# 2thleZ/flash_attention_metal

Hardware: AMD Instinct MI355X
Metric: attn_fwd_tflops (seqlen=4096, head_dim=64, bf16, causal) (higher is better)
Workload: dtype bf16; 1 GPU; BASELINE.json configs[2]: seqlen=4096 head_dim=64 batch=4 heads=16 bf16 is_causal=true per GPU; batch_per_gpu=4, heads=16, seq_len=4096, head_dim=64, is_causal=True

## Files before the change

flash_attention_metal_amd/csrc/fa_mfma16_kernel.hip:

```cpp
#include <stdlib.h>

#include <algorithm>

#include "fa_mfma_common.h"

#ifndef FA16_DEFER_THR
#define FA16_DEFER_THR 8.0f
#endif
#ifndef FA16_LAK
#define FA16_LAK (D == 128 ? 3 : 2)
#endif
#ifndef FA16_LAV
#define FA16_LAV (D == 128 ? 3 : 2)
#endif
#ifndef FA16_PRIO
#define FA16_PRIO 1
#endif
#ifndef FA16_ONES
#define FA16_ONES 1
#endif
#ifndef FA16_HALVES
#define FA16_HALVES 0
#endif
#ifndef FA16_BN128
#define FA16_BN128 64
#endif
#ifndef FA16_OCC128
#define FA16_OCC128 2
#endif
#ifndef FA16_SUB8
#define FA16_SUB8 1
#endif
#ifndef FA16_OCC
#define FA16_OCC 4
#endif

namespace fa {

typedef float f32x4 __attribute__((ext_vector_type(4)));

template <typename Tag> struct MT16;
template <> struct MT16<BF16> {
  using elem = __bf16;
  using vec8 = bf16x8;
  __device__ static __forceinline__ f32x4 mfma(vec8 a, vec8 b, f32x4 c) { return __builtin_amdgcn_mfma_f32_16x16x32_bf16(a, b, c, 0, 0, 0); }
};
template <> struct MT16<F16> {
  using elem = _Float16;
  using vec8 = f16x8;
  __device__ static __forceinline__ f32x4 mfma(vec8 a, vec8 b, f32x4 c) { return __builtin_amdgcn_mfma_f32_16x16x32_f16(a, b, c, 0, 0, 0); }
};

__device__ __forceinline__ float xlane(float x, int mask) { return __shfl_xor(x, mask, 64); }

template <typename Tag, int D, bool CAUSAL, int RW, bool PAD, int SUB>
__device__ __forceinline__ void fwd_mfma16_body(const Params &p) {
  using M = MT16<Tag>;
  using vec8 = typename M::vec8;
  using elem = typename M::elem;
  constexpr int BMR = RW * WM;
  constexpr int RB = D * 2;
  constexpr int CPR = D / 8;
  constexpr int KS = D / 32;
  constexpr int DT = D / 16;
  constexpr int BNK = (D == 128) ? FA16_BN128 : BN;
  constexpr int KT = BNK / 16;
  constexpr int NKP = KT / 2;
  constexpr int TILE = BNK * RB;
  static_assert(D == 64 || D == 128, "head dims of the 16x16x32 kernel");

  extern __shared__ __attribute__((aligned(16))) char smem_generic[];
  lds_char *smem = (lds_char *)smem_generic;
  lds_char *Kbuf = smem;
  lds_char *Vbuf = smem + 2 * SUB * TILE;

  const int wave = __builtin_amdgcn_readfirstlane((int)threadIdx.x >> 6);
  const int lane = threadIdx.x & 63;
  const int c = lane & 15;
  const int g = lane >> 4;

  int bh, qb;
  map_block<CAUSAL>(blockIdx.x, p, bh, qb);
  long long base, base_kv;
  head_bases(bh, p, base, base_kv);
  const int coff = p.Nk - p.N;
  const int q0 = qb * BMR;
  const int qw0 = q0 + wave * WM;

  const int GRB = PAD ? p.D * 2 : RB;
  auto gcol = [&](int chunk) -> unsigned { return (!PAD || chunk * 8 < p.D) ? (unsigned)chunk * 16 : 0x80000000u; };
  const unsigned head_bytes = (unsigned)p.N * GRB, kv_head_bytes = (unsigned)p.Nk * GRB;
  const __amdgpu_buffer_rsrc_t rq = __builtin_amdgcn_make_buffer_rsrc((void *)((const char *)p.q + base * 2), 0, head_bytes, 0x00020000);
  const __amdgpu_buffer_rsrc_t rk = __builtin_amdgcn_make_buffer_rsrc((void *)((const char *)p.k + base_kv * 2), 0, kv_head_bytes, 0x00020000);
  const __amdgpu_buffer_rsrc_t rv = __builtin_amdgcn_make_buffer_rsrc((void *)((const char *)p.v + base_kv * 2), 0, kv_head_bytes, 0x00020000);

  vec8 qf[2][KS];
#pragma unroll
  for (int qt = 0; qt < 2; ++qt)
#pragma unroll
    for (int ks = 0; ks < KS; ++ks) {
      const u32x4 t = __builtin_amdgcn_raw_buffer_load_b128(rq, (unsigned)(qw0 + 16 * qt + c) * GRB + gcol(4 * ks + g), 0, 0);
      qf[qt][ks] = __builtin_bit_cast(vec8, t);
    }

  const int kx = (D == 64) ? ((c >> 1) & 7) : c;
  const lds_char *kptr[KS];
#pragma unroll
  for (int ks = 0; ks < KS; ++ks) {
    kptr[ks] = Kbuf + c * RB + (((4 * ks + g) ^ kx) << 4);
    asm volatile("" : "+v"(kptr[ks]));
  }
  const int vq = c >> 2, vp = c & 3;
  const int vrow = 4 * g + vq;
  const int vx = (D == 64) ? (((vrow >> 1) & 3) << 1) : ((vrow & 7) << 1);
  const lds_char *vptr[DT];
#pragma unroll
  for (int dt = 0; dt < DT; ++dt) {
    vptr[dt] = Vbuf + vrow * RB + ((((2 * dt) ^ vx) + (vp >> 1)) << 4) + 8 * (vp & 1);
    asm volatile("" : "+v"(vptr[dt]));
  }

  const int kv_end = CAUSAL ? min(p.Nk, q0 + BMR + coff) : p.Nk;
  const int nT = (kv_end + BNK - 1) / BNK;

  constexpr int RPP = 1024 / RB;
  constexpr int NPW = (BNK / RPP) / RW;
  static_assert((RW * RPP) % 16 == 0, "the piece stride must keep the swizzle");
  unsigned dma_kvo, dma_vvo;
  {
    const int row = wave * RPP + lane / CPR, pc = lane % CPR;
    const int skx = (D == 64) ? ((row >> 1) & 7) : (row & 15);
    const int svx = (D == 64) ? (((row >> 1) & 3) << 1) : ((row & 7) << 1);
    dma_kvo = (unsigned)(row * GRB) + gcol(pc ^ skx);
    dma_vvo = (unsigned)(row * GRB) + gcol(pc ^ svx);
  }
  auto stage_dma = [&](int t, int buf) {
#pragma unroll
    for (int j = 0; j < NPW; ++j) {
      const unsigned soff = PAD ? (unsigned)(t * BNK + j * RW * RPP) * GRB : (unsigned)t * TILE + j * (RW * 1024);
      const unsigned lk = (unsigned)(__UINTPTR_TYPE__)Kbuf + buf * TILE + (wave + RW * j) * 1024;
      const unsigned lv = (unsigned)(__UINTPTR_TYPE__)Vbuf + buf * TILE + (wave + RW * j) * 1024;
      asm volatile("s_mov_b32 m0, %0\n\ts_nop 0\n\tbuffer_load_dwordx4 %1, %2, %3 offen lds" ::"s"(lk), "v"(dma_kvo), "s"(rk), "s"(soff) : "memory");
      asm volatile("s_mov_b32 m0, %0\n\ts_nop 0\n\tbuffer_load_dwordx4 %1, %2, %3 offen lds" ::"s"(lv), "v"(dma_vvo), "s"(rv), "s"(soff) : "memory");
    }
  };

  f32x4 oacc[DT][2];
#pragma unroll
  for (int dt = 0; dt < DT; ++dt)
#pragma unroll
    for (int qt = 0; qt < 2; ++qt)
#pragma unroll
      for (int i = 0; i < 4; ++i) oacc[dt][qt][i] = 0.0f;
  constexpr bool ONES = (FA16_ONES != 0);
  constexpr float BIAS = !ONES ? 0.0f : std::is_same<Tag, F16>::value ? 3.0f : 7.0f;
  constexpr float FIRST_SUM_FLOOR = std::is_same<Tag, F16>::value ? 1.0f : 0x1p-64f;
  float l[2] = {0.0f, 0.0f};
  f32x4 lacc[2];
#pragma unroll
  for (int qt = 0; qt < 2; ++qt)
#pragma unroll
    for (int i = 0; i < 4; ++i) lacc[qt][i] = 0.0f;
  vec8 ones;
#pragma unroll
  for (int j = 0; j < 8; ++j) ones[j] = (elem)1.0f;
  if constexpr (ONES) asm volatile("" : "+v"(ones));
  const float c2 = p.scale * 1.4426950408889634f;
  f32x4 negm[2];
#pragma unroll
  for (int qt = 0; qt < 2; ++qt) {
#pragma unroll
    for (int i = 0; i < 4; ++i) negm[qt][i] = ONES ? -BIAS : INFINITY;
    asm volatile("" : "+v"(negm[qt]));
  }

  stage_dma(0, 0);
  if constexpr (SUB == 2) {
    if (1 < nT) stage_dma(1, 1);
  }
  asm volatile("s_waitcnt vmcnt(0)" ::: "memory");
#pragma unroll
  for (int qt = 0; qt < 2; ++qt)
#pragma unroll
    for (int ks = 0; ks < KS; ++ks) {
#pragma unroll
      for (int j = 0; j < 8; ++j) qf[qt][ks][j] = (elem)((float)qf[qt][ks][j] * c2);
      asm volatile("" : "+v"(qf[qt][ks]));
    }
  __syncthreads();

  const float sum_thr = __builtin_exp2f(FA16_DEFER_THR);
  auto apply_mask = [&](auto k0c, auto &s, const int kv0) __attribute__((always_inline)) {
    constexpr int K0 = decltype(k0c)::value;
    constexpr int NKT = sizeof(s) / sizeof(s[0]);
    int g4 = 4 * g;
    asm volatile("" : "+v"(g4));
#pragma unroll
    for (int qt = 0; qt < 2; ++qt) {
      int lim = p.Nk - 1 - kv0 - g4;
      if (CAUSAL) lim = min(lim, qw0 + 16 * qt + c + coff - kv0 - g4);
#pragma unroll
      for (int k2 = 0; k2 < NKT; ++k2)
#pragma unroll
        for (int i = 0; i < 4; ++i) s[k2][qt][i] = (16 * (K0 + k2) + i > lim) ? -INFINITY : s[k2][qt][i];
    }
  };
  auto needs_mask = [&](const int kv0) __attribute__((always_inline)) { return (CAUSAL && (kv0 + BNK - 1 > qw0 + coff)) || (kv0 + BNK > p.Nk); };
  auto score_group = [&](auto bufc, auto k0c, auto &s, const f32x4 c0, const f32x4 c1) __attribute__((always_inline)) {
    constexpr int buf = decltype(bufc)::value;
    constexpr int K0 = decltype(k0c)::value;
    constexpr int NKT = sizeof(s) / sizeof(s[0]);
    constexpr int NK = NKT * KS, LA = (FA16_LAK < NK) ? FA16_LAK : NK;
    vec8 kf[NK];
    auto kread = [&](int i) { kf[i] = __builtin_bit_cast(vec8, lds_read_b128(kptr[i % KS] + buf * TILE + (K0 + i / KS) * 16 * RB)); };
#pragma unroll
    for (int i = 0; i < LA; ++i) kread(i);
    __builtin_amdgcn_sched_barrier(0);
#pragma unroll
    for (int i = 0; i < NK; ++i) {
      const int k2 = i / KS, ks = i % KS;
      s[k2][0] = M::mfma(kf[i], qf[0][ks], ks == 0 ? c0 : s[k2][0]);
      s[k2][1] = M::mfma(kf[i], qf[1][ks], ks == 0 ? c1 : s[k2][1]);
      if (i + LA < NK) kread(i + LA);
      __builtin_amdgcn_sched_barrier(0);
    }
  };
  auto pack_group = [&](auto k0c, auto &s, vec8 (&pf)[NKP][2], unsigned &bits) __attribute__((always_inline)) {
    constexpr int K0 = decltype(k0c)::value;
    constexpr int NKT = sizeof(s) / sizeof(s[0]);
#pragma unroll
    for (int kp = 0; kp < NKT / 2; ++kp)
#pragma unroll
      for (int qt = 0; qt < 2; ++qt) {
#pragma unroll
        for (int j = 0; j < 8; ++j) pf[K0 / 2 + kp][qt][j] = (elem)s[2 * kp + (j >> 2)][qt][j & 3];
        if constexpr (ONES) {
          const u32x4 w = __builtin_bit_cast(u32x4, pf[K0 / 2 + kp][qt]);
          bits |= w[0] | w[1] | w[2] | w[3];
        }
      }
  };
  auto hot_group = [&](auto bufc, auto k0c, auto nktc, const int kv0, vec8 (&pf)[NKP][2], unsigned &bits,
                       float (&ls)[2]) __attribute__((always_inline)) {
    constexpr int NKT = decltype(nktc)::value;
    f32x4 s[NKT][2];
    score_group(bufc, k0c, s, negm[0], negm[1]);
    if (needs_mask(kv0)) apply_mask(k0c, s, kv0);
#if FA16_PRIO
    if constexpr (decltype(k0c)::value + NKT == KT) __builtin_amdgcn_s_setprio(0);
#endif
#pragma unroll
    for (int k2 = 0; k2 < NKT; ++k2)
#pragma unroll
      for (int i = 0; i < 4; ++i)
#pragma unroll
        for (int qt = 0; qt < 2; ++qt) {
          s[k2][qt][i] = __builtin_amdgcn_exp2f(s[k2][qt][i]);
          if constexpr (!ONES) ls[qt] = (decltype(k0c)::value == 0 && k2 == 0 && i == 0) ? s[k2][qt][i] : ls[qt] + s[k2][qt][i];
        }
    pack_group(k0c, s, pf, bits);
  };
  auto max_group = [&](auto bufc, auto k0c, auto nktc, const int kv0, float (&mx)[2]) __attribute__((always_inline)) {
    constexpr int NKT = decltype(nktc)::value;
    f32x4 s[NKT][2], zero;
#pragma unroll
    for (int i = 0; i < 4; ++i) zero[i] = 0.0f;
    score_group(bufc, k0c, s, zero, zero);
    if (needs_mask(kv0)) apply_mask(k0c, s, kv0);
#pragma unroll
    for (int qt = 0; qt < 2; ++qt)
#pragma unroll
      for (int k2 = 0; k2 < NKT; ++k2)
#pragma unroll
        for (int i = 0; i < 4; ++i) mx[qt] = fmaxf(mx[qt], s[k2][qt][i]);
  };
  auto new_reference = [&](auto firstc, float (&mx)[2]) __attribute__((always_inline)) {
    constexpr bool FIRST = decltype(firstc)::value;
#pragma unroll
    for (int qt = 0; qt < 2; ++qt) {
      float v = mx[qt];
      v = fmaxf(v, xlane(v, 16));
      v = fmaxf(v, xlane(v, 32));
      const float m_old = -negm[qt][0];
      const float m_new = FIRST ? v + BIAS : fmaxf(m_old, v + BIAS);
#pragma unroll
      for (int i = 0; i < 4; ++i) negm[qt][i] = -m_new;
      asm volatile("" : "+v"(negm[qt]));
      if constexpr (FIRST) continue;
      const float alpha = __builtin_amdgcn_exp2f(m_old - m_new);
      if constexpr (ONES) {
#pragma unroll
        for (int i = 0; i < 4; ++i) lacc[qt][i] *= alpha;
      } else {
        l[qt] *= alpha;
      }
#pragma unroll
      for (int dt = 0; dt < DT; ++dt)
#pragma unroll
        for (int i = 0; i < 4; ++i) oacc[dt][qt][i] *= alpha;
    }
  };
  constexpr int G = (FA16_HALVES != 0) ? 2 : 1;
  using KTG = std::integral_constant<int, KT / G>;
  using K0A = std::integral_constant<int, 0>;
  using K0B = std::integral_constant<int, KT / 2>;

  auto tile = [&](auto bufc, auto firstc, const int t) {
    constexpr int buf = decltype(bufc)::value;
    constexpr bool FIRST = decltype(firstc)::value;
    const int kv0 = t * BNK;

    int always = 1;
    if constexpr (!CAUSAL) asm volatile("" : "+s"(always));
    const bool wave_active = CAUSAL ? (kv0 <= qw0 + WM - 1 + coff) : (always != 0);
    if (wave_active) {
      vec8 pf[NKP][2];
      float ls[2] = {0.0f, 0.0f};
      bool redo = FIRST && !ONES;
      for (;;) {
        if (__builtin_expect(redo, 0)) {
          float mx[2] = {-INFINITY, -INFINITY};
          max_group(bufc, K0A{}, std::integral_constant<int, KT / 2>{}, kv0, mx);
          max_group(bufc, K0B{}, std::integral_constant<int, KT / 2>{}, kv0, mx);
          new_reference(firstc, mx);
        }
#if FA16_PRIO
        __builtin_amdgcn_s_setprio(1);
#endif
        unsigned bits = 0;
        hot_group(bufc, K0A{}, KTG{}, kv0, pf, bits, ls);
        if constexpr (G == 2) hot_group(bufc, K0B{}, KTG{}, kv0, pf, bits, ls);
        bool stale;
        if constexpr (ONES) stale = __builtin_amdgcn_ballot_w64((bits & 0x40004000u) != 0) != 0;
        else stale = __builtin_amdgcn_ballot_w64(fmaxf(ls[0], ls[1]) > sum_thr) != 0;
        if (__builtin_expect(stale && !redo, 0)) {
          redo = true;
          continue;
        }
        if constexpr (!ONES) {
          l[0] += ls[0];
          l[1] += ls[1];
        }
#if FA16_PRIO
        __builtin_amdgcn_s_setprio(1);
#endif
        {
          constexpr int NV = NKP * DT, LA = FA16_LAV;
          s16x4 wlo[NV], whi[NV];
          auto vread = [&](int j) {
            const lds_char *vb = vptr[j % DT] + buf * TILE + (32 * (j / DT)) * RB;
            wlo[j] = lds_read_tr16(vb);
            whi[j] = lds_read_tr16(vb + 16 * RB);
          };
#pragma unroll
          for (int j = 0; j < LA; ++j) vread(j);
          __builtin_amdgcn_sched_barrier(0);
#pragma unroll
          for (int j = 0; j < NV; ++j) {
            const s16x8 v8 = __builtin_shufflevector(wlo[j], whi[j], 0, 1, 2, 3, 4, 5, 6, 7);
#pragma unroll
            for (int qt = 0; qt < 2; ++qt) oacc[j % DT][qt] = M::mfma(__builtin_bit_cast(vec8, v8), pf[j / DT][qt], oacc[j % DT][qt]);
            if (j + LA < NV) vread(j + LA);
            if constexpr (ONES) {
              if (j % DT == DT - 1) {
#pragma unroll
                for (int qt = 0; qt < 2; ++qt) lacc[qt] = M::mfma(ones, pf[j / DT][qt], lacc[qt]);
              }
            }
            __builtin_amdgcn_sched_barrier(0);
          }
        }
#if FA16_PRIO
        __builtin_amdgcn_s_setprio(0);
#endif
        if constexpr (FIRST && ONES) {
          if (__builtin_expect(!redo && __builtin_amdgcn_ballot_w64(fminf(lacc[0][0], lacc[1][0]) < FIRST_SUM_FLOOR) != 0, 0)) {
#pragma unroll
            for (int qt = 0; qt < 2; ++qt) {
#pragma unroll
              for (int i = 0; i < 4; ++i) lacc[qt][i] = 0.0f;
#pragma unroll
              for (int dt = 0; dt < DT; ++dt)
#pragma unroll
                for (int i = 0; i < 4; ++i) oacc[dt][qt][i] = 0.0f;
            }
            redo = true;
            continue;
          }
        }
        break;
      }
    }
  };
  auto unit = [&](auto bufc, auto firstc, const int t0) {
    constexpr int buf = decltype(bufc)::value;
#pragma unroll
    for (int sub = 0; sub < SUB; ++sub)
      if (t0 + SUB + sub < nT) stage_dma(t0 + SUB + sub, (buf ^ 1) * SUB + sub);
    tile(std::integral_constant<int, buf * SUB>{}, firstc, t0);
    if constexpr (SUB == 2) {
      if (t0 + 1 < nT) tile(std::integral_constant<int, buf * SUB + 1>{}, std::false_type{}, t0 + 1);
    }
    if (t0 + SUB < nT) asm volatile("s_waitcnt vmcnt(0)" ::: "memory");
    __syncthreads();
  };
  unit(std::integral_constant<int, 0>{}, std::true_type{}, 0);
  for (int t = SUB; t < nT; t += 2 * SUB) {
    unit(std::integral_constant<int, 1>{}, std::false_type{}, t);
    if (t + SUB < nT) unit(std::integral_constant<int, 0>{}, std::false_type{}, t + SUB);
  }

  lds_char *Ot = smem + wave * (WM * RB);
#pragma unroll
  for (int qt = 0; qt < 2; ++qt) {
    float lt = ONES ? lacc[qt][0] : l[qt];
    if constexpr (!ONES) {
      lt += xlane(lt, 16);
      lt += xlane(lt, 32);
    }
    const float inv_l = __builtin_amdgcn_rcpf(lt);
    const int row = 16 * qt + c, qrow = qw0 + row;
    if (p.lse != nullptr && g == 0 && qrow < p.N)
      p.lse[(long long)bh * p.N + qrow] = (__builtin_amdgcn_logf(lt) - negm[qt][0]) * 0.6931471805599453f;
#pragma unroll
    for (int dt = 0; dt < DT; ++dt) {
      typedef elem elem4 __attribute__((ext_vector_type(4)));
      elem4 e;
#pragma unroll
      for (int i = 0; i < 4; ++i) e[i] = (elem)(oacc[dt][qt][i] * inv_l);
      const u32x2 w = __builtin_bit_cast(u32x2, e);
      const int ch = (2 * dt + (g >> 1)) ^ (row & (CPR - 1));
      lds_write_b64(Ot + row * RB + (ch << 4) + 8 * (g & 1), w);
    }
  }
  __syncthreads();
  {
    elem *Og = (elem *)p.o + base;
#pragma unroll
    for (int it = 0; it < WM * CPR / 64; ++it) {
      const int idx = it * 64 + lane;
      const int row = idx / CPR, ch = idx % CPR;
      const u32x4 vv = lds_read_b128(Ot + row * RB + ((ch ^ (row & (CPR - 1))) << 4));
      if (qw0 + row < p.N && (!PAD || ch * 8 < p.D)) *reinterpret_cast<u32x4 *>(Og + (long long)(qw0 + row) * (PAD ? p.D : D) + ch * 8) = vv;
    }
  }
}

template <typename Tag, int D, bool CAUSAL, int RW, bool PAD = false, int SUB = 1>
__global__ __launch_bounds__(64 * RW, (D == 64 ? FA16_OCC : FA16_OCC128)) void fwd_mfma16_kernel(Params p) {
  fwd_mfma16_body<Tag, D, CAUSAL, RW, PAD, SUB>(p);
}

bool mfma16_supported(int dtype, int D) { return (dtype == FA_DTYPE_F16 || dtype == FA_DTYPE_BF16) && D >= 8 && D <= 128 && D % 8 == 0; }

template <typename Tag, int D, bool CAUSAL, int RW, bool PAD = false, int SUB = 1>
static hipError_t launch16_one(const Params &p, hipStream_t s) {
  const int nQ = (p.N + RW * WM - 1) / (RW * WM);
  const size_t smem = 4 * SUB * (size_t)(D == 128 ? FA16_BN128 : BN) * D * 2;
  auto kern = fwd_mfma16_kernel<Tag, D, CAUSAL, RW, PAD, SUB>;
  if (smem > 48 * 1024) {
    hipError_t e = set_dyn_lds_once((const void *)kern, (int)smem);
    if (e != hipSuccess) return e;
  }
  Params pp = p;
  pp.head_group = causal_head_group(p, D, 2);
#ifdef FA16_FORCE_HEAD_GROUP
  pp.head_group = FA16_FORCE_HEAD_GROUP;
#endif
  set_block_divisors(pp, nQ, pp.head_group);
  (void)hipGetLastError();
  hipLaunchKernelGGL(kern, dim3(nQ * p.B * p.H), dim3(64 * RW), smem, s, pp);
  return hipGetLastError();
}

int mfma16_waves(int D, int BH, int N, int Nk, int is_causal) {
#ifdef FA16_FORCE_RW
  return FA16_FORCE_RW;
#endif
  if (D != 64 && D != 128) return 4;
  const long long b256 = (long long)BH * ((N + 255) / 256);
  if (D == 128) return (!is_causal && Nk >= 8192 && b256 >= 1024) ? 8 : 4;
  if (!is_causal) return (Nk >= 512 && b256 >= 512) ? 8 : 4;
  return (Nk >= 4096 && Nk < 6144 && b256 >= 1024 && b256 < 1280) ? 8 : 4;
}

hipError_t launch_mfma16(const Params &p, int dtype, hipStream_t s) {
  const bool w8 = mfma16_waves(p.D, p.B * p.H, p.N, p.Nk, p.is_causal) == 8 && (p.D == 64 || !p.is_causal);
  auto go = [&](auto tag) -> hipError_t {
    using Tag = decltype(tag);
    if (p.D != 64 && p.D != 128) {
      if (p.D < 64) return p.is_causal ? launch16_one<Tag, 64, true, 4, true>(p, s) : launch16_one<Tag, 64, false, 4, true>(p, s);
      return p.is_causal ? launch16_one<Tag, 128, true, 4, true>(p, s) : launch16_one<Tag, 128, false, 4, true>(p, s);
    }
    if (p.D == 64) {
      if (w8) return p.is_causal ? launch16_one<Tag, 64, true, 8, false, FA16_SUB8>(p, s) : launch16_one<Tag, 64, false, 8, false, FA16_SUB8>(p, s);
      return p.is_causal ? launch16_one<Tag, 64, true, 4>(p, s) : launch16_one<Tag, 64, false, 4>(p, s);
    }
    if (p.D == 128) {
      if (w8) return launch16_one<Tag, 128, false, 8>(p, s);
      return p.is_causal ? launch16_one<Tag, 128, true, 4>(p, s) : launch16_one<Tag, 128, false, 4>(p, s);
    }
    return hipErrorInvalidValue;
  };
  return dtype == FA_DTYPE_F16 ? go(F16{}) : go(BF16{});
}

}
```

Before: 1169 TFLOP/s.

## Interleave causal query rows across waves and skip dead q-tiles per stretch

In the causal path, each wave now takes one 16-row query tile from the front of the block and one from the mirrored back end, which balances causal work across waves. The KV loop is split into three stretches: both q-tiles live, only the late tile live, and none live. Score and PV MFMAs for the finished tile are skipped at compile time, and masking plus first-tile renormalisation are handled per q-tile. Q loads are also issued after the first K/V DMA, and causal w8 is forced to SUB=1. This adds template instantiations and code size, and the strided output rows may coalesce less well.

Result: no change. 1167 TFLOP/s (-0.2%).

```diff
diff --git a/flash_attention_metal_amd/csrc/fa_mfma16_kernel.hip b/flash_attention_metal_amd/csrc/fa_mfma16_kernel.hip
--- a/flash_attention_metal_amd/csrc/fa_mfma16_kernel.hip
+++ b/flash_attention_metal_amd/csrc/fa_mfma16_kernel.hip
@@ -86,6 +86,7 @@
   const int coff = p.Nk - p.N;
   const int q0 = qb * BMR;
   const int qw0 = q0 + wave * WM;
+  auto qrow0 = [&](int qt) { return CAUSAL ? q0 + 16 * (qt == 0 ? wave : 2 * RW - 1 - wave) : qw0 + 16 * qt; };
 
   const int GRB = PAD ? p.D * 2 : RB;
   auto gcol = [&](int chunk) -> unsigned { return (!PAD || chunk * 8 < p.D) ? (unsigned)chunk * 16 : 0x80000000u; };
@@ -95,13 +96,16 @@
   const __amdgpu_buffer_rsrc_t rv = __builtin_amdgcn_make_buffer_rsrc((void *)((const char *)p.v + base_kv * 2), 0, kv_head_bytes, 0x00020000);
 
   vec8 qf[2][KS];
-#pragma unroll
-  for (int qt = 0; qt < 2; ++qt)
-#pragma unroll
-    for (int ks = 0; ks < KS; ++ks) {
-      const u32x4 t = __builtin_amdgcn_raw_buffer_load_b128(rq, (unsigned)(qw0 + 16 * qt + c) * GRB + gcol(4 * ks + g), 0, 0);
-      qf[qt][ks] = __builtin_bit_cast(vec8, t);
-    }
+  constexpr bool DMA_FIRST = CAUSAL;
+  if constexpr (!DMA_FIRST) {
+#pragma unroll
+    for (int qt = 0; qt < 2; ++qt)
+#pragma unroll
+      for (int ks = 0; ks < KS; ++ks) {
+        const u32x4 t = __builtin_amdgcn_raw_buffer_load_b128(rq, (unsigned)(qrow0(qt) + c) * GRB + gcol(4 * ks + g), 0, 0);
+        qf[qt][ks] = __builtin_bit_cast(vec8, t);
+      }
+  }
 
   const int kx = (D == 64) ? ((c >> 1) & 7) : c;
   const lds_char *kptr[KS];
@@ -178,6 +182,16 @@
   if constexpr (SUB == 2) {
     if (1 < nT) stage_dma(1, 1);
   }
+  if constexpr (DMA_FIRST) {
+    __builtin_amdgcn_sched_barrier(0);
+#pragma unroll
+    for (int qt = 0; qt < 2; ++qt)
+#pragma unroll
+      for (int ks = 0; ks < KS; ++ks) {
+        const u32x4 t = __builtin_amdgcn_raw_buffer_load_b128(rq, (unsigned)(qrow0(qt) + c) * GRB + gcol(4 * ks + g), 0, 0);
+        qf[qt][ks] = __builtin_bit_cast(vec8, t);
+      }
+  }
   asm volatile("s_waitcnt vmcnt(0)" ::: "memory");
 #pragma unroll
   for (int qt = 0; qt < 2; ++qt)
@@ -187,26 +201,46 @@
       for (int j = 0; j < 8; ++j) qf[qt][ks][j] = (elem)((float)qf[qt][ks][j] * c2);
       asm volatile("" : "+v"(qf[qt][ks]));
     }
+  if constexpr (DMA_FIRST) {
+    __builtin_amdgcn_sched_barrier(0);
+    if (1 < nT) stage_dma(1, 1);
+  }
   __syncthreads();
 
   const float sum_thr = __builtin_exp2f(FA16_DEFER_THR);
-  auto apply_mask = [&](auto k0c, auto &s, const int kv0) __attribute__((always_inline)) {
+  auto apply_mask = [&](auto qac, auto qbc, auto k0c, auto &s, const int kv0) __attribute__((always_inline)) {
     constexpr int K0 = decltype(k0c)::value;
     constexpr int NKT = sizeof(s) / sizeof(s[0]);
     int g4 = 4 * g;
     asm volatile("" : "+v"(g4));
 #pragma unroll
-    for (int qt = 0; qt < 2; ++qt) {
+    for (int qt = decltype(qac)::value; qt < decltype(qbc)::value; ++qt) {
       int lim = p.Nk - 1 - kv0 - g4;
-      if (CAUSAL) lim = min(lim, qw0 + 16 * qt + c + coff - kv0 - g4);
+      if (CAUSAL) lim = min(lim, qrow0(qt) + c + coff - kv0 - g4);
 #pragma unroll
       for (int k2 = 0; k2 < NKT; ++k2)
 #pragma unroll
         for (int i = 0; i < 4; ++i) s[k2][qt][i] = (16 * (K0 + k2) + i > lim) ? -INFINITY : s[k2][qt][i];
     }
   };
-  auto needs_mask = [&](const int kv0) __attribute__((always_inline)) { return (CAUSAL && (kv0 + BNK - 1 > qw0 + coff)) || (kv0 + BNK > p.Nk); };
-  auto score_group = [&](auto bufc, auto k0c, auto &s, const f32x4 c0, const f32x4 c1) __attribute__((always_inline)) {
+  auto needs_mask = [&](const int qt, const int kv0) __attribute__((always_inline)) { return (CAUSAL && (kv0 + BNK - 1 > qrow0(qt) + coff)) || (kv0 + BNK > p.Nk); };
+  auto mask_live = [&](auto q0c, auto k0c, auto &s, const int kv0) __attribute__((always_inline)) {
+    using QT0 = std::integral_constant<int, 0>;
+    using QT1 = std::integral_constant<int, 1>;
+    using QT2 = std::integral_constant<int, 2>;
+    if constexpr (!CAUSAL) {
+      if (needs_mask(0, kv0)) apply_mask(QT0{}, QT2{}, k0c, s, kv0);
+    } else if constexpr (decltype(q0c)::value == 1) {
+      if (needs_mask(1, kv0)) apply_mask(QT1{}, QT2{}, k0c, s, kv0);
+    } else {
+      if (needs_mask(0, kv0)) {
+        apply_mask(QT0{}, QT1{}, k0c, s, kv0);
+        if (needs_mask(1, kv0)) apply_mask(QT1{}, QT2{}, k0c, s, kv0);
+      }
+    }
+  };
+  auto score_group = [&](auto q0c, auto bufc, auto k0c, auto &s, const f32x4 c0, const f32x4 c1) __attribute__((always_inline)) {
+    constexpr int Q0 = decltype(q0c)::value;
     constexpr int buf = decltype(bufc)::value;
     constexpr int K0 = decltype(k0c)::value;
     constexpr int NKT = sizeof(s) / sizeof(s[0]);
@@ -219,19 +253,19 @@
 #pragma unroll
     for (int i = 0; i < NK; ++i) {
       const int k2 = i / KS, ks = i % KS;
-      s[k2][0] = M::mfma(kf[i], qf[0][ks], ks == 0 ? c0 : s[k2][0]);
+      if constexpr (Q0 == 0) s[k2][0] = M::mfma(kf[i], qf[0][ks], ks == 0 ? c0 : s[k2][0]);
       s[k2][1] = M::mfma(kf[i], qf[1][ks], ks == 0 ? c1 : s[k2][1]);
       if (i + LA < NK) kread(i + LA);
       __builtin_amdgcn_sched_barrier(0);
     }
   };
-  auto pack_group = [&](auto k0c, auto &s, vec8 (&pf)[NKP][2], unsigned &bits) __attribute__((always_inline)) {
+  auto pack_group = [&](auto q0c, auto k0c, auto &s, vec8 (&pf)[NKP][2], unsigned &bits) __attribute__((always_inline)) {
     constexpr int K0 = decltype(k0c)::value;
     constexpr int NKT = sizeof(s) / sizeof(s[0]);
 #pragma unroll
     for (int kp = 0; kp < NKT / 2; ++kp)
 #pragma unroll
-      for (int qt = 0; qt < 2; ++qt) {
+      for (int qt = decltype(q0c)::value; qt < 2; ++qt) {
 #pragma unroll
         for (int j = 0; j < 8; ++j) pf[K0 / 2 + kp][qt][j] = (elem)s[2 * kp + (j >> 2)][qt][j & 3];
         if constexpr (ONES) {
@@ -240,12 +274,12 @@
         }
       }
   };
-  auto hot_group = [&](auto bufc, auto k0c, auto nktc, const int kv0, vec8 (&pf)[NKP][2], unsigned &bits,
+  auto hot_group = [&](auto q0c, auto bufc, auto k0c, auto nktc, const int kv0, vec8 (&pf)[NKP][2], unsigned &bits,
                        float (&ls)[2]) __attribute__((always_inline)) {
     constexpr int NKT = decltype(nktc)::value;
     f32x4 s[NKT][2];
-    score_group(bufc, k0c, s, negm[0], negm[1]);
-    if (needs_mask(kv0)) apply_mask(k0c, s, kv0);
+    score_group(q0c, bufc, k0c, s, negm[0], negm[1]);
+    mask_live(q0c, k0c, s, kv0);
 #if FA16_PRIO
     if constexpr (decltype(k0c)::value + NKT == KT) __builtin_amdgcn_s_setprio(0);
 #endif
@@ -254,30 +288,33 @@
 #pragma unroll
       for (int i = 0; i < 4; ++i)
 #pragma unroll
-        for (int qt = 0; qt < 2; ++qt) {
+        for (int qt = decltype(q0c)::value; qt < 2; ++qt) {
           s[k2][qt][i] = __builtin_amdgcn_exp2f(s[k2][qt][i]);
           if constexpr (!ONES) ls[qt] = (decltype(k0c)::value == 0 && k2 == 0 && i == 0) ? s[k2][qt][i] : ls[qt] + s[k2][qt][i];
         }
-    pack_group(k0c, s, pf, bits);
-  };
-  auto max_group = [&](auto bufc, auto k0c, auto nktc, const int kv0, float (&mx)[2]) __attribute__((always_inline)) {
+    pack_group(q0c, k0c, s, pf, bits);
+  };
+  auto max_group = [&](auto q0c, auto bufc, auto k0c, auto nktc, const int kv0, float (&mx)[2]) __attribute__((always_inline)) {
     constexpr int NKT = decltype(nktc)::value;
     f32x4 s[NKT][2], zero;
 #pragma unroll
     for (int i = 0; i < 4; ++i) zero[i] = 0.0f;
-    score_group(bufc, k0c, s, zero, zero);
-    if (needs_mask(kv0)) apply_mask(k0c, s, kv0);
-#pragma unroll
-    for (int qt = 0; qt < 2; ++qt)
+    score_group(q0c, bufc, k0c, s, zero, zero);
+    mask_live(q0c, k0c, s, kv0);
+#pragma unroll
+    for (int qt = decltype(q0c)::value; qt < 2; ++qt)
 #pragma unroll
       for (int k2 = 0; k2 < NKT; ++k2)
 #pragma unroll
         for (int i = 0; i < 4; ++i) mx[qt] = fmaxf(mx[qt], s[k2][qt][i]);
   };
-  auto new_reference = [&](auto firstc, float (&mx)[2]) __attribute__((always_inline)) {
+  auto new_reference = [&](auto q0c, auto firstc, float (&mx)[2], const bool (&renew)[2]) __attribute__((always_inline)) {
     constexpr bool FIRST = decltype(firstc)::value;
 #pragma unroll
-    for (int qt = 0; qt < 2; ++qt) {
+    for (int qt = decltype(q0c)::value; qt < 2; ++qt) {
+      if constexpr (FIRST && CAUSAL) {
+        if (!renew[qt]) continue;
+      }
       float v = mx[qt];
       v = fmaxf(v, xlane(v, 16));
       v = fmaxf(v, xlane(v, 32));
@@ -305,31 +342,28 @@
   using K0A = std::integral_constant<int, 0>;
   using K0B = std::integral_constant<int, KT / 2>;
 
-  auto tile = [&](auto bufc, auto firstc, const int t) {
+  auto tile_live = [&](auto q0c, auto bufc, auto firstc, const int kv0) __attribute__((always_inline)) {
+    constexpr int Q0 = decltype(q0c)::value;
     constexpr int buf = decltype(bufc)::value;
     constexpr bool FIRST = decltype(firstc)::value;
-    const int kv0 = t * BNK;
-
-    int always = 1;
-    if constexpr (!CAUSAL) asm volatile("" : "+s"(always));
-    const bool wave_active = CAUSAL ? (kv0 <= qw0 + WM - 1 + coff) : (always != 0);
-    if (wave_active) {
+    {
       vec8 pf[NKP][2];
       float ls[2] = {0.0f, 0.0f};
       bool redo = FIRST && !ONES;
+      bool renew[2] = {true, true};
       for (;;) {
         if (__builtin_expect(redo, 0)) {
           float mx[2] = {-INFINITY, -INFINITY};
-          max_group(bufc, K0A{}, std::integral_constant<int, KT / 2>{}, kv0, mx);
-          max_group(bufc, K0B{}, std::integral_constant<int, KT / 2>{}, kv0, mx);
-          new_reference(firstc, mx);
+          max_group(q0c, bufc, K0A{}, std::integral_constant<int, KT / 2>{}, kv0, mx);
+          max_group(q0c, bufc, K0B{}, std::integral_constant<int, KT / 2>{}, kv0, mx);
+          new_reference(q0c, firstc, mx, renew);
         }
 #if FA16_PRIO
         __builtin_amdgcn_s_setprio(1);
 #endif
         unsigned bits = 0;
-        hot_group(bufc, K0A{}, KTG{}, kv0, pf, bits, ls);
-        if constexpr (G == 2) hot_group(bufc, K0B{}, KTG{}, kv0, pf, bits, ls);
+        hot_group(q0c, bufc, K0A{}, KTG{}, kv0, pf, bits, ls);
+        if constexpr (G == 2) hot_group(q0c, bufc, K0B{}, KTG{}, kv0, pf, bits, ls);
         bool stale;
         if constexpr (ONES) stale = __builtin_amdgcn_ballot_w64((bits & 0x40004000u) != 0) != 0;
         else stale = __builtin_amdgcn_ballot_w64(fmaxf(ls[0], ls[1]) > sum_thr) != 0;
@@ -359,12 +393,12 @@
           for (int j = 0; j < NV; ++j) {
             const s16x8 v8 = __builtin_shufflevector(wlo[j], whi[j], 0, 1, 2, 3, 4, 5, 6, 7);
 #pragma unroll
-            for (int qt = 0; qt < 2; ++qt) oacc[j % DT][qt] = M::mfma(__builtin_bit_cast(vec8, v8), pf[j / DT][qt], oacc[j % DT][qt]);
+            for (int qt = Q0; qt < 2; ++qt) oacc[j % DT][qt] = M::mfma(__builtin_bit_cast(vec8, v8), pf[j / DT][qt], oacc[j % DT][qt]);
             if (j + LA < NV) vread(j + LA);
             if constexpr (ONES) {
               if (j % DT == DT - 1) {
 #pragma unroll
-                for (int qt = 0; qt < 2; ++qt) lacc[qt] = M::mfma(ones, pf[j / DT][qt], lacc[qt]);
+                for (int qt = Q0; qt < 2; ++qt) lacc[qt] = M::mfma(ones, pf[j / DT][qt], lacc[qt]);
               }
             }
             __builtin_amdgcn_sched_barrier(0);
@@ -374,7 +408,25 @@
         __builtin_amdgcn_s_setprio(0);
 #endif
         if constexpr (FIRST && ONES) {
-          if (__builtin_expect(!redo && __builtin_amdgcn_ballot_w64(fminf(lacc[0][0], lacc[1][0]) < FIRST_SUM_FLOOR) != 0, 0)) {
+          if constexpr (CAUSAL) {
+            if (!redo) {
+              renew[0] = __builtin_amdgcn_ballot_w64(lacc[0][0] < FIRST_SUM_FLOOR) != 0;
+              renew[1] = __builtin_amdgcn_ballot_w64(lacc[1][0] < FIRST_SUM_FLOOR) != 0;
+            }
+            if (__builtin_expect(!redo && (renew[0] || renew[1]), 0)) {
+#pragma unroll
+              for (int qt = 0; qt < 2; ++qt) {
+#pragma unroll
+                for (int i = 0; i < 4; ++i) lacc[qt][i] = 0.0f;
+#pragma unroll
+                for (int dt = 0; dt < DT; ++dt)
+#pragma unroll
+                  for (int i = 0; i < 4; ++i) oacc[dt][qt][i] = 0.0f;
+              }
+              redo = true;
+              continue;
+            }
+          } else if (__builtin_expect(!redo && __builtin_amdgcn_ballot_w64(fminf(lacc[0][0], lacc[1][0]) < FIRST_SUM_FLOOR) != 0, 0)) {
 #pragma unroll
             for (int qt = 0; qt < 2; ++qt) {
 #pragma unroll
@@ -392,22 +444,60 @@
       }
     }
   };
-  auto unit = [&](auto bufc, auto firstc, const int t0) {
+  auto tile = [&](auto q0c, auto bufc, auto firstc, const int t) {
+    constexpr bool FIRST = decltype(firstc)::value;
+    const int kv0 = t * BNK;
+    if constexpr (!CAUSAL) {
+      int always = 1;
+      asm volatile("" : "+s"(always));
+      if (always != 0) tile_live(q0c, bufc, firstc, kv0);
+    } else if constexpr (FIRST) {
+      if (kv0 <= qrow0(1) + 15 + coff) tile_live(q0c, bufc, firstc, kv0);
+    } else if constexpr (decltype(q0c)::value < 2) {
+      tile_live(q0c, bufc, firstc, kv0);
+    }
+  };
+  auto unit = [&](auto q0c, auto bufc, auto firstc, const int t0) {
     constexpr int buf = decltype(bufc)::value;
 #pragma unroll
-    for (int sub = 0; sub < SUB; ++sub)
+    for (int sub = 0; sub < SUB; ++sub) {
+      if constexpr (DMA_FIRST && decltype(firstc)::value) continue;
       if (t0 + SUB + sub < nT) stage_dma(t0 + SUB + sub, (buf ^ 1) * SUB + sub);
-    tile(std::integral_constant<int, buf * SUB>{}, firstc, t0);
+    }
+    tile(q0c, std::integral_constant<int, buf * SUB>{}, firstc, t0);
     if constexpr (SUB == 2) {
-      if (t0 + 1 < nT) tile(std::integral_constant<int, buf * SUB + 1>{}, std::false_type{}, t0 + 1);
+      if (t0 + 1 < nT) tile(q0c, std::integral_constant<int, buf * SUB + 1>{}, std::false_type{}, t0 + 1);
     }
     if (t0 + SUB < nT) asm volatile("s_waitcnt vmcnt(0)" ::: "memory");
     __syncthreads();
   };
-  unit(std::integral_constant<int, 0>{}, std::true_type{}, 0);
-  for (int t = SUB; t < nT; t += 2 * SUB) {
-    unit(std::integral_constant<int, 1>{}, std::false_type{}, t);
-    if (t + SUB < nT) unit(std::integral_constant<int, 0>{}, std::false_type{}, t + SUB);
+  using QBOTH = std::integral_constant<int, 0>;
+  using BUF0 = std::integral_constant<int, 0>;
+  using BUF1 = std::integral_constant<int, 1>;
+  unit(QBOTH{}, BUF0{}, std::true_type{}, 0);
+  if constexpr (!CAUSAL) {
+    for (int t = SUB; t < nT; t += 2 * SUB) {
+      unit(QBOTH{}, BUF1{}, std::false_type{}, t);
+      if (t + SUB < nT) unit(QBOTH{}, BUF0{}, std::false_type{}, t + SUB);
+    }
+  } else {
+    static_assert(SUB == 1, "the causal stretches are counted in tiles");
+    const int tA = max(1, min(nT, (qrow0(0) + 15 + coff + BNK) / BNK));
+    const int tB = max(tA, min(nT, (qrow0(1) + 15 + coff + BNK) / BNK));
+    for (int t = 1; t < tA; t += 2) {
+      unit(QBOTH{}, BUF1{}, std::false_type{}, t);
+      if (t + 1 < tA) unit(QBOTH{}, BUF0{}, std::false_type{}, t + 1);
+    }
+    using QLATE = std::integral_constant<int, 1>;
+    for (int t = tA; t < tB; ++t) {
+      if (t & 1) unit(QLATE{}, BUF1{}, std::false_type{}, t);
+      else unit(QLATE{}, BUF0{}, std::false_type{}, t);
+    }
+    using QNONE = std::integral_constant<int, 2>;
+    for (int t = tB; t < nT; ++t) {
+      if (t & 1) unit(QNONE{}, BUF1{}, std::false_type{}, t);
+      else unit(QNONE{}, BUF0{}, std::false_type{}, t);
+    }
   }
 
   lds_char *Ot = smem + wave * (WM * RB);
@@ -419,7 +509,7 @@
       lt += xlane(lt, 32);
     }
     const float inv_l = __builtin_amdgcn_rcpf(lt);
-    const int row = 16 * qt + c, qrow = qw0 + row;
+    const int row = 16 * qt + c, qrow = CAUSAL ? qrow0(qt) + c : qw0 + row;
     if (p.lse != nullptr && g == 0 && qrow < p.N)
       p.lse[(long long)bh * p.N + qrow] = (__builtin_amdgcn_logf(lt) - negm[qt][0]) * 0.6931471805599453f;
 #pragma unroll
@@ -441,7 +531,12 @@
       const int idx = it * 64 + lane;
       const int row = idx / CPR, ch = idx % CPR;
       const u32x4 vv = lds_read_b128(Ot + row * RB + ((ch ^ (row & (CPR - 1))) << 4));
-      if (qw0 + row < p.N && (!PAD || ch * 8 < p.D)) *reinterpret_cast<u32x4 *>(Og + (long long)(qw0 + row) * (PAD ? p.D : D) + ch * 8) = vv;
+      if constexpr (CAUSAL) {
+        const int qrow = qrow0(row >> 4) + (row & 15);
+        if (qrow < p.N && (!PAD || ch * 8 < p.D)) *reinterpret_cast<u32x4 *>(Og + (long long)qrow * (PAD ? p.D : D) + ch * 8) = vv;
+      } else {
+        if (qw0 + row < p.N && (!PAD || ch * 8 < p.D)) *reinterpret_cast<u32x4 *>(Og + (long long)(qw0 + row) * (PAD ? p.D : D) + ch * 8) = vv;
+      }
     }
   }
 }
@@ -493,7 +588,7 @@
       return p.is_causal ? launch16_one<Tag, 128, true, 4, true>(p, s) : launch16_one<Tag, 128, false, 4, true>(p, s);
     }
     if (p.D == 64) {
-      if (w8) return p.is_causal ? launch16_one<Tag, 64, true, 8, false, FA16_SUB8>(p, s) : launch16_one<Tag, 64, false, 8, false, FA16_SUB8>(p, s);
+      if (w8) return p.is_causal ? launch16_one<Tag, 64, true, 8>(p, s) : launch16_one<Tag, 64, false, 8, false, FA16_SUB8>(p, s);
       return p.is_causal ? launch16_one<Tag, 64, true, 4>(p, s) : launch16_one<Tag, 64, false, 4>(p, s);
     }
     if (p.D == 128) {
```
